# nullmax-vision/SimPB

Measured on AMD Instinct MI355X. Metric: frames/sec (6-cam sample) + MSDeformAttn HBM GB/s, R50 704x256 @1/2/4/8 GPU, higher is better.
Workload: dtype f32

## Files before the change

### include/simpb_hip.h

```cpp
#ifndef SIMPB_HIP_H
#define SIMPB_HIP_H

#ifdef __cplusplus
extern "C" {
#endif

#define SIMPB_OK 0
#define SIMPB_EINVAL 1
#define SIMPB_ELAUNCH 2

#define SIMPB_RECORD3D_WIDTH 15

int simpb_abi_version(void);

const char* simpb_last_error(void);

#define SIMPB_KERNEL_DAF 1
#define SIMPB_KERNEL_MSDA 2
int simpb_timing_enable(int capacity);
int simpb_timing_read(int kernel_id, float* ms_out, int max_n);
void simpb_timing_reset(void);

int simpb_deformable_aggregation_forward(
    float* output, const float* mc_ms_feat, const int* spatial_shape, const int* scale_start_index,
// ... 80 lines not shown
int simpb_preprocess_mid_pitch(int out_width);

#define SIMPB_GEMM_MAX_SEGS 4
#define SIMPB_GEMM_MAX_JOBS 4
#define SIMPB_GEMM_OUT_F32 0
#define SIMPB_GEMM_OUT_SPLIT_HALFS 1
typedef struct simpb_gemm_job {
  const float* x[SIMPB_GEMM_MAX_SEGS];
  int ldx[SIMPB_GEMM_MAX_SEGS];
  int kseg[SIMPB_GEMM_MAX_SEGS];
  int num_seg;
  int M, N, K;
  const float* w;
  const float* bias;
  float* y;
  const int* m_live;
  int ldw, ldy, relu;
  int out_fmt;
  const int* row_flag;
  const float* bias2;
  const void* w_hi;
  const void* w_lo;
} simpb_gemm_job;
typedef struct simpb_gemm_args {
  int num_jobs;
  int reserved;
  simpb_gemm_job job[SIMPB_GEMM_MAX_JOBS];
} simpb_gemm_args;
int simpb_gemm_f32(const simpb_gemm_args* args, void* stream);

int simpb_layernorm_f32(float* out, int ldo, const float* x0, int ld0, int k0, const float* x1, int ld1, int k1,
                        const float* gamma, const float* beta, int num_rows, const int* m_live, void* stream);

#define SIMPB_MAX_LEVELS 8
int simpb_format_tokens(float* col_feats, const void* const* level_ptrs, const void* const* level_bias,
                        const int* level_hw, int num_levels, int num_images, int channels, int src_is_half, void* stream);

int simpb_bias_act_nhwc_f16(void* y, const void* bias, const void* residual, long long num_pixels, int channels,
                            int relu, void* stream);

int simpb_bias_relu_maxpool_nhwc_f16(void* y, const void* x, const void* bias, int num_images, int in_h, int in_w,
                                     int channels, void* stream);

int simpb_conv1x1_nhwc_f16(void* y, const void* x, const void* weight, const void* bias, const void* residual,
                           int num_images, int in_h, int in_w, int in_channels, int out_channels, int stride, int relu,
                           int residual_upsample2x, const void* input_bias, int variant, void* stream);

int simpb_conv3x3_nhwc_f16(void* y, float* tokens, void* tokens_f16, int tokens_per_cam, int level_start, const void* x,
                           const void* weight, const void* bias, int num_images, int in_h, int in_w, int in_channels,
                           int out_channels, int stride, int relu, int variant, void* stream);

int simpb_conv3x3_choose_variant(long long p_out, int in_channels, int out_channels);

int simpb_conv3x3_group_tokens_f16(int num_levels, float* tokens, void* tokens_f16, int tokens_per_cam, const int* level_start,
                                   const void* const* x, const void* const* weight, const void* const* bias, int num_images,
                                   const int* in_h, const int* in_w, int in_channels, int out_channels, int relu, void* stream);

int simpb_attention_f32(float* out, const float* q, const float* k, const float* v, const int* query_cam,
                        const int* group_start, int batch_size, int num_heads, int head_dim, int num_query,
                        int num_key, int ldq, int ldk, int ldv, int ldo, float scale, void* stream);

int simpb_attention_f32_split(float* out, const float* q, const float* k, const float* v, const int* query_cam,
                              const int* group_start, int batch_size, int num_heads, int head_dim, int num_query,
                              int num_key, int ldq, int ldk, int ldv, int ldo, float scale, void* stream);

int simpb_attention_split_halfs(float* out, const void* q, const void* k, const void* v, const int* query_cam,
                                const int* group_start, int batch_size, int num_heads, int head_dim, int num_query,
                                int num_key, int ldq, int ldk, int ldv, int ldo, void* stream);

#define SIMPB_MLP_MAX_OPS 12
#define SIMPB_MLP_MAX_CHAINS 8
#define SIMPB_MLP_POST_NONE 0
#define SIMPB_MLP_POST_REFINE3D 1
#define SIMPB_MLP_POST_REFINE2D 2
#define SIMPB_MLP_POST_SIGMOID 3
#define SIMPB_MLP_LINEAR 0
#define SIMPB_MLP_LAYERNORM 1
#define SIMPB_MLP_IN_ROWS 0
#define SIMPB_MLP_IN_SINE2D 1
#define SIMPB_MLP_IN_ROWS_LN 2
typedef struct simpb_mlp_op {
  int type, in_dim, out_dim, relu;
  const float* w;
  const float* b;
} simpb_mlp_op;
typedef struct simpb_mlp_chain {
  const float* x;
  const float* x2;
  float* out;
  const float* out_scale;
  int ldx, ldx2, ldo, in_dim, in_mode, n_ops;
  int post, ldres, res_cols, div_rows, div_col0, reserved;
  const float* res;
  const float* div;
  simpb_mlp_op ops[SIMPB_MLP_MAX_OPS];
  const float* ln_w;
  const float* ln_b;
  float* ln_out;
  int ld_ln_out, reserved2;
} simpb_mlp_chain;
typedef struct simpb_mlp_args {
  int num_rows, num_chains;
  int weights_transposed;
  int reserved;
  simpb_mlp_chain chain[SIMPB_MLP_MAX_CHAINS];
  const int* m_live;
} simpb_mlp_args;
int simpb_mlp_chain_forward(const simpb_mlp_args* args, void* stream);

// ... 157 lines not shown
```

### simpb_amd/_lib.py

```python
import ctypes
import os

from .build import LIB

_lib = None

_P = ctypes.c_void_p
_I = ctypes.c_int
_F = ctypes.c_float
_LL = ctypes.c_longlong


class WorldTables(ctypes.Structure):
    _fields_ = [("class_range", _F * 32), ("attr_moving", ctypes.c_ubyte * 32), ("attr_still", ctypes.c_ubyte * 32),
                ("threshold", _F), ("has_threshold", _I), ("num_output", _I)]


SIGNATURES = {
    "simpb_abi_version": ([], _I),
    "simpb_last_error": ([], ctypes.c_char_p),
    "simpb_timing_enable": ([_I], _I),
    "simpb_timing_read": ([_I, _P, _I], _I),
    "simpb_timing_reset": ([], None),
    "simpb_deformable_aggregation_forward": ([_P] * 6 + [_I] * 8 + [_P], _I),
    "simpb_dfa_fused_forward": ([_P, _P, _I] + [_P] * 11 + [_I] * 9 + [_P], _I),
    "simpb_dfa_fused_forward_cams": ([_P, _P, _I] + [_P] * 11 + [_I] * 9 + [_P, _P], _I),
    "simpb_deformable_aggregation_backward": ([_P] * 9 + [_I] * 8 + [_P], _I),
    "simpb_ms_deform_attn_grouped_forward": ([_P] * 7 + [_I] * 8 + [_P], _I),
    "simpb_msda_linear_forward": ([_P, _I, _P, _I, _P, _P, _P, _I, _P, _I, _P, _P] + [_I] * 8 + [_P], _I),
    "simpb_ms_deform_attn_grouped_backward": ([_P] * 10 + [_I] * 8 + [_P], _I),
    "simpb_linear_f32": ([_P] * 4 + [_I] * 4 + [_P], _I),
    "simpb_linear_f16x3": ([_P] * 5 + [_I] * 3 + [_P], _I),
    "simpb_gemm_f32": ([_P, _P], _I),
    "simpb_layernorm_f32": ([_P, _I, _P, _I, _I, _P, _I, _I, _P, _P, _I, _P, _P], _I),
    "simpb_bias_act_nhwc_f16": ([_P, _P, _P, ctypes.c_longlong, _I, _I, _P], _I),
    "simpb_bias_relu_maxpool_nhwc_f16": ([_P, _P, _P, _I, _I, _I, _I, _P], _I),
    "simpb_conv1x1_nhwc_f16": ([_P] * 5 + [_I] * 8 + [_P, _I, _P], _I),
    "simpb_conv3x3_nhwc_f16": ([_P, _P, _P, _I, _I, _P, _P, _P] + [_I] * 8 + [_P], _I),
    "simpb_conv3x3_choose_variant": ([_LL, _I, _I], _I),
    "simpb_conv3x3_group_tokens_f16": ([_I, _P, _P, _I, _P, _P, _P, _P, _I, _P, _P, _I, _I, _I, _P], _I),
    "simpb_stem_conv7x7_pool_f16": ([_P] * 4 + [_I] * 4 + [_P], _I),
    "simpb_image_to_nhwc4_f16": ([_P, _P] + [ctypes.c_longlong] * 4 + [_I] * 4 + [_P], _I),
    "simpb_preprocess_u8_nhwc4_f16": ([_P] * 10 + [_I] * 11 + [_P], _I),
    "simpb_preprocess_yuv420sp_nhwc4_f16": ([_P] * 10 + [_I] * 18 + [_P], _I),
    "simpb_preprocess_surface_nhwc4_f16": ([_P] * 11 + [_I] * 12 + [_LL] * 4 + [_I] * 6 + [_P], _I),
    "simpb_preprocess_mid_pitch": ([_I], _I),
    "simpb_linear_f16in_split": ([_P] * 5 + [_I] * 3 + [_P], _I),
    "simpb_format_tokens": ([_P, _P, _P, _P, _I, _I, _I, _I, _P], _I),
    "simpb_attention_f32": ([_P] * 6 + [_I] * 9 + [_F, _P], _I),
    "simpb_attention_f32_split": ([_P] * 6 + [_I] * 9 + [_F, _P], _I),
    "simpb_attention_split_halfs": ([_P] * 6 + [_I] * 9 + [_P], _I),
    "simpb_mlp_chain_forward": ([_P, _P], _I),
    "simpb_bank_get": ([_P] * 6 + [_I] * 2 + [_F] * 2 + [_P], _I),
    "simpb_bank_update": ([_P] * 10 + [_I] * 5 + [_P], _I),
    "simpb_bank_update_rank": ([_P, _P] + [_I] * 4 + [_P], _I),
    "simpb_bank_update_merge": ([_P] * 13 + [_I, _P] + [_I] * 5 + [_P], _I),
    "simpb_bank_update_merge_active": ([_P] * 13 + [_I, _P] + [_I] * 5 + [_P, _P], _I),
    "simpb_bank_cache": ([_P] * 10 + [_I] * 6 + [_F, _I, _F, _P, _I, _P, _P], _I),
    "simpb_bank_cache_streams": ([_P] * 10 + [_I] * 6 + [_F, _I, _F, _P, _I, _P, _P, _P], _I),
    "simpb_bank_cache_streams_active": ([_P] * 10 + [_I] * 6 + [_F, _I, _F, _P, _I, _P, _P, _P, _P], _I),
    "simpb_decode3d_record": ([_P] * 6 + [_I] * 4 + [_P], _I),
    "simpb_decode2d_record": ([_P] * 6 + [_I] * 4 + [_F] * 4 + [_P], _I),
    "simpb_record2d_compact": ([_P, _LL, _P, _LL, _I, _I, _I, _P], _I),
    "simpb_decode2d_record_ragged": ([_P] * 7 + [_I] * 5 + [_F] * 4 + [_P], _I),
    "simpb_world_record": ([_P] * 5 + [WorldTables, _I, _P], _I),
    "simpb_topk_rows": ([_P, _P, _P, _I, _I, _I, _P], _I),
    "simpb_rowdot_sigmoid": ([_P, _P, _I, _P, _P, _I, _I, _P, _P], _I),
    "simpb_anchor_projection": ([_P] * 4 + [_I] * 2 + [_P], _I),
    "simpb_msda_prep": ([_P, _P, _P, _I, _P, _I, _P, _I, _I, _I, _I, _P, _P], _I),
    "simpb_dfa_points": ([_P] * 7 + [_I] * 5 + [_P], _I),
    "simpb_dfa_weights": ([_P] * 3 + [_I] * 6 + [_P], _I),
    "simpb_dfa_points_cams": ([_P] * 7 + [_I] * 5 + [_P, _P], _I),
    "simpb_dfa_weights_cams": ([_P] * 3 + [_I] * 6 + [_P, _P], _I),
    "simpb_alloc_project_cams": ([_P] * 5 + [_I] * 3 + [_F] * 5 + [_P, _P], _I),
    "simpb_alloc_project": ([_P] * 5 + [_I] * 3 + [_F] * 5 + [_P], _I),
    "simpb_alloc_compact": ([_P] * 3 + [_I] * 3 + [_P], _I),
    "simpb_alloc_group_start": ([_P] * 3 + [_I] * 3 + [_P], _I),
    "simpb_alloc_scatter": ([_P] * 12 + [_I] * 4 + [_F] * 2 + [_P], _I),
    "simpb_alloc_static": ([_P] * 15 + [_I] * 4 + [_F] * 5 + [_P], _I),
    "simpb_alloc_ragged": ([_P] * 15 + [_I] * 4 + [_F] * 5 + [_P], _I),
    "simpb_alloc_ragged_active": ([_P] * 15 + [_I] * 4 + [_F] * 5 + [_P, _P], _I),
    "simpb_alloc_static_cams": ([_P] * 15 + [_I] * 4 + [_F] * 5 + [_P, _P], _I),
    "simpb_alloc_ragged_cams": ([_P] * 15 + [_I] * 4 + [_F] * 5 + [_P, _P, _P], _I),
    "simpb_gather_rows": ([_P] * 3 + [_I] * 4 + [_P], _I),
    "simpb_aggregate_2d_to_3d": ([_P] * 8 + [_I] * 5 + [_P], _I),
    "simpb_aggregate_2d_to_3d_alpha": ([_P] * 9 + [_I, _I, _P, _P] + [_I] * 5 + [_P], _I),
}

ERRORS = {1: "SIMPB_EINVAL (bad pointer/size/layout)", 2: "SIMPB_ELAUNCH (kernel launch failed)"}


def lib():
    global _lib
# ... 22 lines not shown
```

### simpb_amd/csrc/conv3x3.hip

```cpp
#include <hip/hip_runtime.h>
#include <hip/hip_fp16.h>
#include <type_traits>
#include "../../include/simpb_hip.h"
#include "mfma_f16.h"

extern "C" int simpb_check_launch(void);

namespace {

using f32x16 = __attribute__((ext_vector_type(16))) float;
using h16x8 = __attribute__((ext_vector_type(8))) _Float16;

constexpr int BN = 64, BK = 64;
constexpr int LDH = BK + 8;
constexpr int LDC = BN + 1;
constexpr int kThreads = 256;
constexpr int kStageBytes = 2 * BN * LDH * 2;
constexpr int kTileBytes = 4 * 32 * LDC * 4;
constexpr int kSmemBytes = kStageBytes > kTileBytes ? kStageBytes : kTileBytes;

struct ConvArgs {
  _Float16* y;
  float* tok;
  _Float16* tok16;
  const _Float16 *x, *w, *bias;
  const _Float16* residual;
  int res_up;
  int P_out, Cin, Cout, relu, stride, Ho, Wo, H, W;
  int tokens_per_cam, level_start;
  int gx, gy, per_xcd;
};

template <int S>
using IC = std::integral_constant<int, S>;

template <bool TOK16>
__device__ __forceinline__ void emit_piece(const ConvArgs& a, int c0, bool full, int p, int c8, const float (&v)[8]) {
  if (p >= a.P_out) return;
  size_t trow = 0;
  if (TOK16 || a.tok) {
    const int hw = a.Ho * a.Wo;
    const int n = p / hw, pix = p - n * hw;
    trow = ((size_t)n * a.tokens_per_cam + a.level_start + pix) * a.Cout;
  }
  size_t rrow = 0;
  if (a.residual) {
    int rp = p;
    if (a.res_up) {
      const int hw = a.Ho * a.Wo;
      const int n = p / hw, rem = p - n * hw;
      const int ho = rem / a.Wo, wo = rem - ho * a.Wo;
      rp = (n * (a.Ho >> 1) + (ho >> 1)) * (a.Wo >> 1) + (wo >> 1);
    }
    rrow = (size_t)rp * a.Cout;
  }
  if (full) {
    const h16x8 bv = *reinterpret_cast<const h16x8*>(a.bias + c0 + c8);
    h16x8 rv = {0, 0, 0, 0, 0, 0, 0, 0};
    if (a.residual) rv = *reinterpret_cast<const h16x8*>(a.residual + rrow + c0 + c8);
    h16x8 o;
#pragma unroll
    for (int e = 0; e < 8; ++e) {
      const float t = v[e] + (float)bv[e] + (float)rv[e];
      o[e] = (_Float16)(a.relu ? fmaxf(t, 0.f) : t);
    }
    if constexpr (TOK16) {
      *reinterpret_cast<h16x8*>(a.tok16 + trow + c0 + c8) = o;
    } else if (a.tok) {
      float* d = a.tok + trow + c0 + c8;
      *reinterpret_cast<float4*>(d) = make_float4((float)o[0], (float)o[1], (float)o[2], (float)o[3]);
      *reinterpret_cast<float4*>(d + 4) = make_float4((float)o[4], (float)o[5], (float)o[6], (float)o[7]);
      if (a.tok16) *reinterpret_cast<h16x8*>(a.tok16 + trow + c0 + c8) = o;
    } else {
      *reinterpret_cast<h16x8*>(a.y + (size_t)p * a.Cout + c0 + c8) = o;
    }
  } else {
#pragma unroll
    for (int e = 0; e < 8; ++e) {
      const int c = c0 + c8 + e;
      if (c < a.Cout) {
        float t = v[e] + (float)a.bias[c];
        if (a.residual) t += (float)a.residual[rrow + c];
        const _Float16 o = (_Float16)(a.relu ? fmaxf(t, 0.f) : t);
// ... 406 lines not shown
}

template <int BMt, int BNt, int WGM, int WGN, int TAPS, bool TOK16>
__global__ __launch_bounds__(64 * WGM * WGN, WGM * WGN == 3 ? 3 : 2) void conv_staged_kernel(const ConvArgs a) {
  const int tile = (blockIdx.x & 7) * a.per_xcd + (blockIdx.x >> 3);
  if ((int)(blockIdx.x >> 3) >= a.per_xcd || tile >= a.gx * a.gy) return;
  conv_staged_tile<BMt, BNt, WGM, WGN, TAPS, TOK16>(a, tile);
}

template <int BMt, int BNt, int WGM, int WGN, int TAPS, bool TOK16, int KS>
__global__ __launch_bounds__(64 * WGM * WGN * KS, 2) void conv_staged_ksplit_kernel(const ConvArgs a) {
  const int tile = (blockIdx.x & 7) * a.per_xcd + (blockIdx.x >> 3);
  if ((int)(blockIdx.x >> 3) >= a.per_xcd || tile >= a.gx * a.gy) return;
  conv_staged_tile<BMt, BNt, WGM, WGN, TAPS, TOK16, KS, true>(a, tile);
}

constexpr int kMaxConvGroup = 4;
struct ConvGroup {
  ConvArgs a[kMaxConvGroup];
  int start[kMaxConvGroup + 1];
  int n, per_xcd;
};
template <int BMt, int BNt, int WGM, int WGN, int TAPS, bool TOK16>
__global__ __launch_bounds__(64 * WGM * WGN, WGM * WGN == 3 ? 3 : 2) void conv_staged_group_kernel(const ConvGroup g) {
  const int gt = (blockIdx.x & 7) * g.per_xcd + (blockIdx.x >> 3);
  if ((int)(blockIdx.x >> 3) >= g.per_xcd || gt >= g.start[g.n]) return;
  int j = 0;
#pragma unroll
  for (int t = 1; t < kMaxConvGroup; ++t)
    if (t < g.n && gt >= g.start[t]) j = t;
  conv_staged_tile<BMt, BNt, WGM, WGN, TAPS, TOK16>(g.a[j], gt - g.start[j]);
}

template <int BMt, int BNt, int WGM, int WGN, int TAPS, bool TOK16>
void launch_staged(ConvArgs& a, hipStream_t stream) {
  a.gx = (a.P_out + BMt - 1) / BMt;
  a.gy = (a.Cout + BNt - 1) / BNt;
  const long long total = (long long)a.gx * a.gy;
  a.per_xcd = (int)((total + 7) / 8);
  hipLaunchKernelGGL((conv_staged_kernel<BMt, BNt, WGM, WGN, TAPS, TOK16>), dim3((unsigned)(a.per_xcd * 8)), dim3(64 * WGM * WGN), 0,
                     stream, a);
}

template <int BMt, int BNt, int WGM, int WGN, int TAPS, bool TOK16, int KS>
void launch_staged_ksplit(ConvArgs& a, hipStream_t stream) {
  a.gx = (a.P_out + BMt - 1) / BMt;
  a.gy = (a.Cout + BNt - 1) / BNt;
  const long long total = (long long)a.gx * a.gy;
  a.per_xcd = (int)((total + 7) / 8);
  hipLaunchKernelGGL((conv_staged_ksplit_kernel<BMt, BNt, WGM, WGN, TAPS, TOK16, KS>), dim3((unsigned)(a.per_xcd * 8)),
                     dim3(64 * WGM * WGN * KS), 0, stream, a);
}

}

extern "C" int simpb_conv3x3_choose_variant(long long p_out, int in_channels, int out_channels) {
  const long long ny = (out_channels + BN - 1) / BN;
  const long long t96 = (p_out + 95) / 96, t128 = (p_out + 127) / 128, t64 = (p_out + 63) / 64;
  if (out_channels >= 128 && t128 * ((out_channels + 127) / 128) >= 2048) return 6;
  if (out_channels >= 128 && t96 * ((out_channels + 127) / 128) >= 160) return 8;
  if (t96 * ny >= 256) return 7;
  if (t128 * ny >= 128) return in_channels >= 256 && out_channels >= 256 ? 9 : 1;
  if (t64 * ny >= 128) return in_channels >= 512 && out_channels >= 512 ? 11 : 4;
  return 3;
}

extern "C" int simpb_conv3x3_nhwc_f16(void* y, float* tokens, void* tokens_f16, int tokens_per_cam, int level_start,
                                      const void* x, const void* weight, const void* bias, int num_images, int in_h, int in_w,
                                      int in_channels, int out_channels, int stride, int relu, int variant, void* stream) {
  const bool to_tokens = tokens || tokens_f16;
  if ((!y && !to_tokens) || (y && to_tokens) || (reinterpret_cast<size_t>(tokens_f16) & 15) || !x || !weight || !bias || num_images <= 0 || in_h <= 0 || in_w <= 0 ||
      in_channels <= 0 || out_channels <= 0 || (stride != 1 && stride != 2) || in_channels % BK != 0 || out_channels % 8 != 0 ||
      variant < 0 || variant > 11)
    return SIMPB_EINVAL;
  if ((reinterpret_cast<size_t>(y) | reinterpret_cast<size_t>(tokens) | reinterpret_cast<size_t>(x) |
       reinterpret_cast<size_t>(weight) | reinterpret_cast<size_t>(bias)) & 15)
    return SIMPB_EINVAL;
  const int ho = (in_h - 1) / stride + 1, wo = (in_w - 1) / stride + 1;
  const long long p_out = (long long)num_images * ho * wo;
  const long long in_elems = (long long)num_images * in_h * in_w * in_channels;
  if (p_out > (1ll << 30) || in_elems > (1ll << 31) - 1) return SIMPB_EINVAL;
  if (to_tokens && (tokens_per_cam < ho * wo || level_start < 0 || level_start + ho * wo > tokens_per_cam)) return SIMPB_EINVAL;
  (void)hipGetLastError();
  ConvArgs a{static_cast<_Float16*>(y), tokens, static_cast<_Float16*>(tokens_f16), static_cast<const _Float16*>(x), static_cast<const _Float16*>(weight),
             static_cast<const _Float16*>(bias), nullptr, 0, (int)p_out, in_channels, out_channels, relu, stride, ho, wo, in_h, in_w,
             tokens_per_cam, level_start, 0, 0, 0};
  if (variant == 0) variant = simpb_conv3x3_choose_variant(p_out, in_channels, out_channels);
  hipStream_t s = static_cast<hipStream_t>(stream);
  auto dispatch = [&](auto tok16_c) {
    constexpr bool T = decltype(tok16_c)::value;
    switch (variant) {
      case 1: launch<1, false, T>(a, s); break;
      case 2: launch<2, false, T>(a, s); break;
      case 3: launch<1, true, T>(a, s); break;
      case 4: launch<2, true, T>(a, s); break;
      case 5: launch_staged<128, 64, 4, 1, 9, T>(a, s); break;
      case 6: launch_staged<128, 128, 2, 2, 9, T>(a, s); break;
      case 7: launch_staged<96, 64, 3, 1, 9, T>(a, s); break;
      case 8: launch_staged<96, 128, 1, 4, 9, T>(a, s); break;
      case 9: launch_staged_ksplit<64, 64, 2, 2, 9, T, 1>(a, s); break;
      case 10: launch_staged_ksplit<64, 64, 2, 2, 9, T, 2>(a, s); break;
      default: launch_staged_ksplit<64, 64, 2, 2, 9, T, 4>(a, s); break;
    }
  };
  if (!tokens && tokens_f16) dispatch(std::true_type{});
  else dispatch(std::false_type{});
  return simpb_check_launch();
}

extern "C" int simpb_conv3x3_group_tokens_f16(int num_levels, float* tokens, void* tokens_f16, int tokens_per_cam,
                                              const int* level_start, const void* const* x, const void* const* weight,
                                              const void* const* bias, int num_images, const int* in_h, const int* in_w,
                                              int in_channels, int out_channels, int relu, void* stream) {
  if (num_levels < 1 || num_levels > kMaxConvGroup || (!tokens && !tokens_f16) || !level_start || !x || !weight || !bias || !in_h || !in_w ||
      num_images <= 0 || in_channels <= 0 || out_channels <= 0 || in_channels % BK != 0 || out_channels % 8 != 0 ||
      ((reinterpret_cast<size_t>(tokens) | reinterpret_cast<size_t>(tokens_f16)) & 15))
    return SIMPB_EINVAL;
  ConvGroup g{};
  long long total = 0;
  for (int j = 0; j < num_levels; ++j) {
    if (!x[j] || !weight[j] || !bias[j] || in_h[j] <= 0 || in_w[j] <= 0 ||
        ((reinterpret_cast<size_t>(x[j]) | reinterpret_cast<size_t>(weight[j]) | reinterpret_cast<size_t>(bias[j])) & 15))
      return SIMPB_EINVAL;
    const long long p_out = (long long)num_images * in_h[j] * in_w[j];
    if (p_out > (1ll << 30) || p_out * in_channels > (1ll << 31) - 1) return SIMPB_EINVAL;
    if (tokens_per_cam < in_h[j] * in_w[j] || level_start[j] < 0 || level_start[j] + in_h[j] * in_w[j] > tokens_per_cam)
      return SIMPB_EINVAL;
    g.a[j] = ConvArgs{nullptr, tokens, static_cast<_Float16*>(tokens_f16), static_cast<const _Float16*>(x[j]),
                      static_cast<const _Float16*>(weight[j]), static_cast<const _Float16*>(bias[j]), nullptr, 0, (int)p_out,
                      in_channels, out_channels, relu, 1, in_h[j], in_w[j], in_h[j], in_w[j], tokens_per_cam, level_start[j],
                      0, 0, 0};
    g.a[j].gx = (int)((p_out + 95) / 96);
    g.a[j].gy = (out_channels + 127) / 128;
    g.start[j] = (int)total;
    total += (long long)g.a[j].gx * g.a[j].gy;
  }
  if (total > (1 << 24)) return SIMPB_EINVAL;
  for (int j = num_levels; j <= kMaxConvGroup; ++j) g.start[j] = (int)total;
  g.n = num_levels;
  g.per_xcd = (int)((total + 7) / 8);
  (void)hipGetLastError();
  if (!tokens)
    hipLaunchKernelGGL((conv_staged_group_kernel<96, 128, 1, 4, 9, true>), dim3((unsigned)(g.per_xcd * 8)), dim3(256), 0,
                       static_cast<hipStream_t>(stream), g);
  else
    hipLaunchKernelGGL((conv_staged_group_kernel<96, 128, 1, 4, 9, false>), dim3((unsigned)(g.per_xcd * 8)), dim3(256), 0,
                       static_cast<hipStream_t>(stream), g);
  return simpb_check_launch();
}

extern "C" int simpb_conv_pointwise_staged(void* y, const void* x, const void* weight, const void* bias, const void* residual,
                                           int p_out, int in_h, int in_w, int ho, int wo, int in_channels, int out_channels,
                                           int stride, int relu, int residual_upsample2x, int tiling, void* stream) {
  ConvArgs a{static_cast<_Float16*>(y), nullptr, nullptr, static_cast<const _Float16*>(x), static_cast<const _Float16*>(weight),
             static_cast<const _Float16*>(bias), static_cast<const _Float16*>(residual), residual_upsample2x ? 1 : 0,
             p_out, in_channels, out_channels, relu, stride, ho, wo, in_h, in_w, 0, 0, 0, 0, 0};
  hipStream_t s = static_cast<hipStream_t>(stream);
  if (tiling == 0) launch_staged<128, 64, 4, 1, 1, false>(a, s);
  else if (tiling == 1) launch_staged<128, 128, 2, 2, 1, false>(a, s);
  else launch_staged<64, 64, 2, 2, 1, false>(a, s);
  return simpb_check_launch();
}
```

### simpb_amd/plugin/ops.py

```python
import ctypes

import torch
from torch.autograd.function import Function

from .. import _lib


def _ptr(t):
    return ctypes.c_void_p(t.data_ptr())


def _stream():
    return ctypes.c_void_p(torch.cuda.current_stream().cuda_stream)


def _require_gpu(*tensors):
    for t in tensors:
        if not t.is_cuda:
            raise RuntimeError("simpb_amd operators run on the GPU only (got a CPU tensor); "
                               "there is no CPU fallback")


_layout_ok = {}

# ... 399 lines not shown
        raise ValueError("residual must match the output (channels_last f16)")
    if input_bias is not None and (input_bias.dtype != torch.float16 or input_bias.numel() != cin or not input_bias.is_contiguous()):
        raise ValueError("input_bias must be a contiguous f16 [Cin] tensor")
    w2 = weight.reshape(cout, cin)
    if not w2.is_contiguous():
        w2 = w2.contiguous()
    status = _lib.lib().simpb_conv1x1_nhwc_f16(_ptr(y), _ptr(x), _ptr(w2), _ptr(bias), _ptr(residual) if residual is not None else None,
                                               n, h, w, cin, cout, stride, 1 if relu else 0,
                                               1 if residual_upsample2x else 0,
                                               _ptr(input_bias) if input_bias is not None else None, variant, _stream())
    _lib.check(status, "simpb_conv1x1_nhwc_f16")
    return y


def conv3x3_nhwc(x, weight, bias, relu=True, stride=1, tokens=None, variant=0):
    _require_gpu(x, weight, bias)
    n, cin, h, w = x.shape
    cout = weight.shape[0]
    if (x.dtype != torch.float16 or not x.is_contiguous(memory_format=torch.channels_last) or weight.dtype != torch.float16
            or bias.dtype != torch.float16 or tuple(weight.shape) != (cout, cin, 3, 3) or cin % 64 or cout % 8
            or stride not in (1, 2) or bias.numel() != cout or not bias.is_contiguous()):
        raise ValueError("conv3x3_nhwc takes channels_last f16 input, f16 [Cout, Cin, 3, 3] weight, Cin % 64 == 0, Cout % 8 == 0")
    if not weight.is_contiguous(memory_format=torch.channels_last):
        weight = weight.contiguous(memory_format=torch.channels_last)
    ho, wo = (h - 1) // stride + 1, (w - 1) // stride + 1
    col16 = None
    if tokens is None:
        y = torch.empty((n, cout, ho, wo), device=x.device, dtype=torch.float16, memory_format=torch.channels_last)
        col, per_cam, start = None, 0, 0
    else:
        col, per_cam, start = tokens[:3]
        col16 = tokens[3] if len(tokens) > 3 else None
        y = None
        if col is None and col16 is None:
            raise ValueError("tokens: an f32 or an f16 token buffer")
        if col16 is not None and (col16.dtype != torch.float16 or not col16.is_contiguous()
                                  or (col is not None and col16.shape != col.shape)):
            raise ValueError("tokens: the f16 buffer must match col_feats")
        rows = col if col is not None else col16
        if ((col is not None and col.dtype != torch.float32) or not rows.is_contiguous() or rows.shape[-1] != cout
                or rows.numel() != n * per_cam * cout or start < 0 or start + ho * wo > per_cam):
            raise ValueError("tokens: (contiguous f32 [bs, cams * tokens_per_cam, Cout] with bs * cams == N, tokens_per_cam, level_start)")
    status = _lib.lib().simpb_conv3x3_nhwc_f16(_ptr(y) if y is not None else None, _ptr(col) if col is not None else None,
                                               _ptr(col16) if col16 is not None else None, per_cam, start, _ptr(x), _ptr(weight), _ptr(bias), n, h, w, cin, cout, stride,
                                               1 if relu else 0, variant, _stream())
    _lib.check(status, "simpb_conv3x3_nhwc_f16")
    return y


def conv3x3_variant_for(p_out, in_channels, out_channels):
    return int(_lib.lib().simpb_conv3x3_choose_variant(int(p_out), int(in_channels), int(out_channels)))


def conv3x3_group_tokens(xs, weights, biases, col, per_cam, starts, col16=None, relu=False):
    import ctypes
    if col is None and col16 is None:
        raise ValueError("conv3x3_group_tokens: an f32 or an f16 token buffer")
    rows = col if col is not None else col16
    _require_gpu(*xs, *weights, *biases, rows)
    n, cin = xs[0].shape[:2]
    cout = weights[0].shape[0]
    k = len(xs)
    if not (1 <= k <= 4 and len(weights) == k and len(biases) == k and len(starts) == k):
        raise ValueError("conv3x3_group_tokens: 1..4 levels, one weight / bias / start each")
    ws = []
    for x, w, b in zip(xs, weights, biases):
        if (x.dtype != torch.float16 or not x.is_contiguous(memory_format=torch.channels_last) or x.shape[0] != n or x.shape[1] != cin
                or w.dtype != torch.float16 or tuple(w.shape) != (cout, cin, 3, 3) or b.dtype != torch.float16 or b.numel() != cout
                or not b.is_contiguous() or cin % 64 or cout % 8):
            raise ValueError("conv3x3_group_tokens takes channels_last f16 inputs of one channel count, f16 [Cout, Cin, 3, 3] weights")
        ws.append(w if w.is_contiguous(memory_format=torch.channels_last) else w.contiguous(memory_format=torch.channels_last))
    if ((col is not None and col.dtype != torch.float32) or not rows.is_contiguous() or rows.shape[-1] != cout
            or rows.numel() != n * per_cam * cout
            or (col16 is not None and (col16.dtype != torch.float16 or not col16.is_contiguous() or col16.shape != rows.shape))):
        raise ValueError("conv3x3_group_tokens: col = contiguous f32 [bs, cams * tokens_per_cam, Cout] with bs * cams == N")
    arr_p, arr_i = ctypes.c_void_p * k, ctypes.c_int * k
    status = _lib.lib().simpb_conv3x3_group_tokens_f16(
        k, _ptr(col) if col is not None else None, _ptr(col16) if col16 is not None else None, int(per_cam), arr_i(*[int(v) for v in starts]),
        arr_p(*[x.data_ptr() for x in xs]), arr_p(*[w.data_ptr() for w in ws]), arr_p(*[b.data_ptr() for b in biases]), n,
        arr_i(*[x.shape[2] for x in xs]), arr_i(*[x.shape[3] for x in xs]), cin, cout, 1 if relu else 0, _stream())
    _lib.check(status, "simpb_conv3x3_group_tokens_f16")


def _stem_weight_packed(weight):
    tag = (weight.data_ptr(), weight._version, str(weight.device))
    hit = getattr(weight, "_simpb_stem_pack", None)
    if hit is None or hit[0] != tag:
        with torch.no_grad():
            w = weight.detach().float()
            full = torch.zeros(64, 4, 7, 8, device=w.device)
            full[:, :3, :, :7] = w
            pack = full.reshape(64, 4, 7, 4, 2).permute(2, 3, 4, 0, 1).contiguous().half()
        hit = (tag, pack)
        weight._simpb_stem_pack = hit
    return hit[1]


def stem_conv_pool(img, weight, bias):
    _require_gpu(img, weight, bias)
    n, c, h, w = img.shape
    if img.dtype != torch.float32 or c != 3 or tuple(weight.shape) != (64, 3, 7, 7) or bias.numel() != 64 or h < 1 or w < 1:
        raise ValueError("stem_conv_pool: f32 [N, 3, H, W] image, [64, 3, 7, 7] weight, 64 biases")
    lib = _lib.lib()
    x4 = torch.empty(n, h, w, 4, device=img.device, dtype=torch.float16)
    _lib.check(lib.simpb_image_to_nhwc4_f16(_ptr(x4), _ptr(img), img.stride(0), img.stride(1), img.stride(2), img.stride(3), n, c, h, w,
                                            _stream()), "simpb_image_to_nhwc4_f16")
    return stem_conv_pool_nhwc4(x4, weight, bias)


def stem_conv_pool_nhwc4(x4, weight, bias):
    _require_gpu(x4, weight, bias)
    if (x4.dtype != torch.float16 or x4.dim() != 4 or x4.shape[3] != 4 or not x4.is_contiguous() or tuple(weight.shape) != (64, 3, 7, 7)
            or bias.numel() != 64 or x4.shape[1] < 1 or x4.shape[2] < 1):
        raise ValueError("stem_conv_pool_nhwc4: contiguous f16 [N, H, W, 4] image, [64, 3, 7, 7] weight, 64 biases")
    n, h, w, _ = x4.shape
    lib = _lib.lib()
    ho, wo = (h - 1) // 2 + 1, (w - 1) // 2 + 1
    hp, wp = (ho - 1) // 2 + 1, (wo - 1) // 2 + 1
    out = torch.empty((n, 64, hp, wp), device=x4.device, dtype=torch.float16, memory_format=torch.channels_last)
    b16 = bias if bias.dtype == torch.float16 and bias.is_contiguous() else bias.half().contiguous()
    _lib.check(lib.simpb_stem_conv7x7_pool_f16(_ptr(out), _ptr(x4), _ptr(_stem_weight_packed(weight)), _ptr(b16), n, h, w, 64,
                                               _stream()), "simpb_stem_conv7x7_pool_f16")
    return out


def preprocess_frames(frames, plan, out=None):
    return plan.run(frames, out=out)


def topk_rows(scores, k):
    _require_gpu(scores)
    if scores.dim() != 2 or scores.shape[1] > 2048:
        raise ValueError("topk_rows takes [bs, n <= 2048] scores")
    scores = scores.contiguous().float()
# ... 47 lines not shown
```

Baseline: 429.0.

## Add LDS-resident halo-tile conv3x3 kernel with per-level group dispatch

Adds a new conv3x3 implicit-GEMM kernel that loads a spatial tile with its halo and the full input-channel depth into LDS once, then reuses it across all nine taps while streaming weight chunks through a 2-3 deep LDS ring. The group-tokens path now picks between this resident form and the existing staged kernel per level, using a heuristic based on tile count, and launches up to two kernels. The aim is to stop re-reading overlapping input pixels from global memory for every tap. The cost is heavy LDS use, which can lower occupancy, plus an extra launch when levels are split between the two forms.

```diff
diff --git a/include/simpb_hip.h b/include/simpb_hip.h
--- a/include/simpb_hip.h
+++ b/include/simpb_hip.h
@@ -156,9 +156,19 @@
 
 int simpb_conv3x3_choose_variant(long long p_out, int in_channels, int out_channels);
 
+int simpb_conv3x3_choose_resident(long long p_out, int in_h, int in_w, int in_channels, int out_channels, int stride);
+
+int simpb_conv3x3_group_choose_resident(int num_levels, int num_images, const int* in_h, const int* in_w, int in_channels,
+                                        int out_channels);
+
 int simpb_conv3x3_group_tokens_f16(int num_levels, float* tokens, void* tokens_f16, int tokens_per_cam, const int* level_start,
                                    const void* const* x, const void* const* weight, const void* const* bias, int num_images,
                                    const int* in_h, const int* in_w, int in_channels, int out_channels, int relu, void* stream);
+
+int simpb_conv3x3_group_tokens_forms_f16(int num_levels, float* tokens, void* tokens_f16, int tokens_per_cam,
+                                         const int* level_start, const void* const* x, const void* const* weight,
+                                         const void* const* bias, int num_images, const int* in_h, const int* in_w,
+                                         int in_channels, int out_channels, int relu, const int* variant, void* stream);
 
 int simpb_attention_f32(float* out, const float* q, const float* k, const float* v, const int* query_cam,
                         const int* group_start, int batch_size, int num_heads, int head_dim, int num_query,
diff --git a/simpb_amd/_lib.py b/simpb_amd/_lib.py
--- a/simpb_amd/_lib.py
+++ b/simpb_amd/_lib.py
@@ -39,6 +39,9 @@
     "simpb_conv3x3_nhwc_f16": ([_P, _P, _P, _I, _I, _P, _P, _P] + [_I] * 8 + [_P], _I),
     "simpb_conv3x3_choose_variant": ([_LL, _I, _I], _I),
     "simpb_conv3x3_group_tokens_f16": ([_I, _P, _P, _I, _P, _P, _P, _P, _I, _P, _P, _I, _I, _I, _P], _I),
+    "simpb_conv3x3_choose_resident": ([_LL, _I, _I, _I, _I, _I], _I),
+    "simpb_conv3x3_group_choose_resident": ([_I, _I, _P, _P, _I, _I], _I),
+    "simpb_conv3x3_group_tokens_forms_f16": ([_I, _P, _P, _I, _P, _P, _P, _P, _I, _P, _P, _I, _I, _I, _P, _P], _I),
     "simpb_stem_conv7x7_pool_f16": ([_P] * 4 + [_I] * 4 + [_P], _I),
     "simpb_image_to_nhwc4_f16": ([_P, _P] + [ctypes.c_longlong] * 4 + [_I] * 4 + [_P], _I),
     "simpb_preprocess_u8_nhwc4_f16": ([_P] * 10 + [_I] * 11 + [_P], _I),
diff --git a/simpb_amd/csrc/conv3x3.hip b/simpb_amd/csrc/conv3x3.hip
--- a/simpb_amd/csrc/conv3x3.hip
+++ b/simpb_amd/csrc/conv3x3.hip
@@ -29,6 +29,7 @@
   int P_out, Cin, Cout, relu, stride, Ho, Wo, H, W;
   int tokens_per_cam, level_start;
   int gx, gy, per_xcd;
+  int tiles_w, tiles_h;
 };
 
 template <int S>
@@ -541,6 +542,281 @@
                      dim3(64 * WGM * WGN * KS), 0, stream, a);
 }
 
+constexpr int RTW = 16, RHW = RTW + 2;
+constexpr int resident_row_bytes(int cin) { return (RHW * (2 * cin + 16) + 255) & ~255; }
+
+template <int CIN, int TH, int BNt, int WGM, int WGN, int RING>
+constexpr size_t resident_lds() {
+  const size_t run = (size_t)(TH + 2) * resident_row_bytes(CIN) + RING * BNt * LDH * 2;
+  const size_t tile = (size_t)WGM * WGN * 32 * (BNt / WGN + 1) * 4;
+  return run > tile ? run : tile;
+}
+
+template <int CIN, int TH, int BNt, int WGM, int WGN, int RING, bool TOK16>
+__device__ __forceinline__ void conv_resident_tile(const ConvArgs& a, const int tile, unsigned char* smem) {
+  constexpr int NT = 64 * WGM * WGN;
+  constexpr int AF = TH * RTW / WGM / 32, NF = BNt / WGN / 32;
+  static_assert(AF * WGM * 32 == TH * RTW && NF * WGN * 32 == BNt && NF <= 2, "tile = waves x 32-row / 32-column fragments");
+  static_assert(CIN == 64 || CIN == 128 || CIN == 256, "the whole Cin is resident");
+  static_assert(RING == 2 || RING == 3, "weight chunks in LDS");
+  constexpr int D = RING - 1;
+  constexpr int PT = CIN / BK, NCH = 9 * PT;
+  constexpr int HEAD = PT <= 2 ? 3 : 6;
+  constexpr int NB = (BNt * 8 + NT - 1) / NT;
+  constexpr int LDW = 32 * NF + 1;
+  constexpr int HP = (TH + 2) * RHW;
+  constexpr int NH = (HP * 8 + NT - 1) / NT;
+  constexpr int PIX = 2 * CIN + 16, ROW = resident_row_bytes(CIN);
+  constexpr int WBUF = BNt * LDH;
+  _Float16* s_b = reinterpret_cast<_Float16*>(smem + (TH + 2) * ROW);
+  float* s_c = reinterpret_cast<float*>(smem);
+  const int W = a.W, H = a.H;
+
+  const int tx = tile / a.gy, ty = tile - tx * a.gy;
+  const int per_img = a.tiles_w * a.tiles_h;
+  const int img = tx / per_img, t2 = tx - img * per_img;
+  const int trow = t2 / a.tiles_w;
+  const int y0 = trow * TH, x0 = (t2 - trow * a.tiles_w) * RTW;
+  const int tid = threadIdx.x;
+  const int lane = tid & 63, wave = tid >> 6;
+  const int r32 = lane & 31, kb = lane >> 5;
+  const int wm = wave / WGN, wn = wave - wm * WGN;
+  const int c0 = ty * BNt;
+  constexpr size_t K = (size_t)9 * CIN;
+  const _Float16* __restrict__ wgt = a.w;
+  const h16x8 zero = {0, 0, 0, 0, 0, 0, 0, 0};
+
+  const int sc = (tid & 7) * 8;
+  size_t brow[NB];
+#pragma unroll
+  for (int i = 0; i < NB; ++i) brow[i] = (size_t)min(c0 + ((tid + NT * i) >> 3), a.Cout - 1) * K + sc;
+  h16x8 rb[3][NB];
+  auto fetch = [&](auto set_c, int chunk) __attribute__((always_inline)) {
+    constexpr int s = decltype(set_c)::value;
+    const size_t koff = (size_t)min(chunk, NCH - 1) * BK;
+#pragma unroll
+    for (int i = 0; i < NB; ++i) rb[s][i] = *reinterpret_cast<const h16x8*>(wgt + brow[i] + koff);
+  };
+  auto stash = [&](auto set_c, int buf) __attribute__((always_inline)) {
+    constexpr int s = decltype(set_c)::value;
+#pragma unroll
+    for (int i = 0; i < NB; ++i) {
+      const int idx = tid + NT * i;
+      if ((BNt * 8) % NT == 0 || idx < BNt * 8) *reinterpret_cast<h16x8*>(&s_b[buf * WBUF + (idx >> 3) * LDH + sc]) = rb[s][i];
+    }
+  };
+
+  fetch(IC<0>{}, 0);
+  fetch(IC<1>{}, 1);
+  fetch(IC<2>{}, 2);
+  h16x8 hv[PT][NH];
+  {
+    const _Float16* __restrict__ src = a.x + (size_t)img * H * W * CIN;
+#pragma unroll
+    for (int i = 0; i < NH; ++i) {
+      const int idx = tid + NT * i;
+      const int hp = idx >> 3;
+      const int hy = hp / RHW, hx = hp - hy * RHW;
+      const int iy = y0 - 1 + hy, ix = x0 - 1 + hx;
+      const bool in = ((HP * 8) % NT == 0 || idx < HP * 8) && iy >= 0 && iy < H && ix >= 0 && ix < W;
+      const _Float16* from = src + ((size_t)iy * W + ix) * CIN + sc;
+#pragma unroll
+      for (int s = 0; s < PT; ++s) {
+        hv[s][i] = zero;
+        if (in) hv[s][i] = *reinterpret_cast<const h16x8*>(from + s * BK);
+      }
+    }
+  }
+  auto halo_to_lds = [&](auto slice_c) __attribute__((always_inline)) {
+    constexpr int s = decltype(slice_c)::value;
+#pragma unroll
+    for (int i = 0; i < NH; ++i) {
+      const int idx = tid + NT * i;
+      const int hp = idx >> 3;
+      const int hy = hp / RHW, hx = hp - hy * RHW;
+      if ((HP * 8) % NT == 0 || idx < HP * 8) *reinterpret_cast<h16x8*>(smem + hy * ROW + hx * PIX + s * (2 * BK) + 2 * sc) = hv[s][i];
+    }
+  };
+  __builtin_amdgcn_sched_barrier(0);
+  stash(IC<0>{}, 0);
+  fetch(IC<0>{}, 3);
+  if constexpr (D == 2) {
+    stash(IC<1>{}, 1);
+    fetch(IC<1>{}, 4);
+  }
+  halo_to_lds(IC<0>{});
+  __syncthreads();
+
+  f32x16 acc[AF][NF];
+#pragma unroll
+  for (int f = 0; f < AF; ++f)
+#pragma unroll
+    for (int n = 0; n < NF; ++n)
+#pragma unroll
+      for (int r = 0; r < 16; ++r) acc[f][n][r] = 0.f;
+
+  const unsigned char* a_lane = smem + (wm * AF * 2 + (r32 >> 4)) * ROW + (r32 & 15) * PIX + 16 * kb;
+  const _Float16* b_lane = s_b + (wn * NF * 32 + r32) * LDH + 8 * kb;
+  h16x8 av[AF], bv[NF];
+  auto pixels = [&](int c, int ks) __attribute__((always_inline)) {
+    const int tap = c / PT, k0 = (c - tap * PT) * BK;
+    const int dy = tap / 3, dx = tap - dy * 3;
+    const unsigned char* sa = a_lane + dy * ROW + dx * PIX + 2 * k0 + 32 * ks;
+#pragma unroll
+    for (int f = 0; f < AF; ++f) av[f] = *reinterpret_cast<const h16x8*>(sa + f * 2 * ROW);
+  };
+  auto weights = [&](int c, int ks) __attribute__((always_inline)) {
+    const _Float16* sb = b_lane + (c % RING) * WBUF + 16 * ks;
+#pragma unroll
+    for (int n = 0; n < NF; ++n) bv[n] = *reinterpret_cast<const h16x8*>(sb + n * 32 * LDH);
+  };
+  auto step = [&](auto set_c, int c, bool ahead, bool read_ahead) __attribute__((always_inline)) {
+    stash(set_c, (c + D) % RING);
+    fetch(set_c, c + D + 3);
+    if constexpr (PT > 1) {
+      if (c == 0) halo_to_lds(IC<1>{});
+    }
+    if constexpr (PT > 2) {
+      if (c == 1) halo_to_lds(IC<2>{});
+      if (c == 2) halo_to_lds(IC<3>{});
+    }
+    __builtin_amdgcn_sched_barrier(0);
+    if (!ahead) pixels(c, 0);
+    if (!ahead || D == 1) weights(c, 0);
+#pragma unroll
+    for (int ks = 0; ks < BK / 16; ++ks) {
+      h16x8 ca[AF], cb[NF];
+#pragma unroll
+      for (int f = 0; f < AF; ++f) ca[f] = av[f];
+#pragma unroll
+      for (int n = 0; n < NF; ++n) cb[n] = bv[n];
+      if (ks + 1 < BK / 16) {
+        pixels(c, ks + 1);
+        weights(c, ks + 1);
+      } else if (read_ahead) {
+        pixels(min(c + 1, NCH - 1), 0);
+        if constexpr (D == 2) weights(min(c + 1, NCH - 1), 0);
+      }
+#pragma unroll
+      for (int f = 0; f < AF; ++f)
+#pragma unroll
+        for (int n = 0; n < NF; ++n) acc[f][n] = simpb::mfma_32x32x16_f16(ca[f], cb[n], acc[f][n]);
+    }
+    __syncthreads();
+  };
+  using S0 = IC<D % 3>;
+  using S1 = IC<(D + 1) % 3>;
+  using S2 = IC<(D + 2) % 3>;
+  step(S0{}, 0, false, 1 >= PT);
+  step(S1{}, 1, 1 >= PT, 2 >= PT);
+  step(S2{}, 2, 2 >= PT, 3 >= PT);
+  if constexpr (HEAD == 6) {
+    step(S0{}, 3, 3 >= PT, true);
+    step(S1{}, 4, true, true);
+    step(S2{}, 5, true, true);
+  }
+  for (int c = HEAD; c < NCH; c += 3) {
+    step(S0{}, c, true, true);
+    step(S1{}, c + 1, true, true);
+    step(S2{}, c + 2, true, true);
+  }
+
+  float* mine = s_c + wave * 32 * LDW;
+  const int cw = c0 + wn * NF * 32;
+  const bool full = cw + 32 * NF <= a.Cout;
+#pragma unroll
+  for (int f = 0; f < AF; ++f) {
+    if (f) __syncthreads();
+#pragma unroll
+    for (int n = 0; n < NF; ++n)
+#pragma unroll
+      for (int r = 0; r < 16; ++r) mine[((r & 3) + 8 * (r >> 2) + 4 * kb) * LDW + n * 32 + r32] = acc[f][n][r];
+    __syncthreads();
+    constexpr int PR = 4 * NF;
+#pragma unroll
+    for (int pass = 0; pass < 32 * PR / 64; ++pass) {
+      const int idx = lane + 64 * pass;
+      const int r = idx / PR, c8 = (idx % PR) * 8;
+      float v[8];
+#pragma unroll
+      for (int e = 0; e < 8; ++e) v[e] = mine[r * LDW + c8 + e];
+      const int oy = y0 + (wm * AF + f) * 2 + (r >> 4), ox = x0 + (r & 15);
+      const int p = oy < H && ox < W ? (img * H + oy) * W + ox : a.P_out;
+      emit_piece<TOK16>(a, cw, full, p, c8, v);
+    }
+  }
+}
+
+template <int CIN, int TH, int BNt, int WGM, int WGN, int RING, bool TOK16>
+__global__ __launch_bounds__(64 * WGM * WGN) void conv_resident_kernel(const ConvArgs a) {
+  extern __shared__ __attribute__((aligned(16))) unsigned char resident_smem[];
+  const int tile = (blockIdx.x & 7) * a.per_xcd + (blockIdx.x >> 3);
+  if ((int)(blockIdx.x >> 3) >= a.per_xcd || tile >= a.gx * a.gy) return;
+  conv_resident_tile<CIN, TH, BNt, WGM, WGN, RING, TOK16>(a, tile, resident_smem);
+}
+
+template <int CIN, int TH, int BNt, int WGM, int WGN, int RING, bool TOK16>
+__global__ __launch_bounds__(64 * WGM * WGN) void conv_resident_group_kernel(const ConvGroup g) {
+  extern __shared__ __attribute__((aligned(16))) unsigned char resident_smem[];
+  const int gt = (blockIdx.x & 7) * g.per_xcd + (blockIdx.x >> 3);
+  if ((int)(blockIdx.x >> 3) >= g.per_xcd || gt >= g.start[g.n]) return;
+  int j = 0;
+#pragma unroll
+  for (int t = 1; t < kMaxConvGroup; ++t)
+    if (t < g.n && gt >= g.start[t]) j = t;
+  conv_resident_tile<CIN, TH, BNt, WGM, WGN, RING, TOK16>(g.a[j], gt - g.start[j], resident_smem);
+}
+
+inline bool resident_shape(int cin, int stride) { return stride == 1 && (cin == 64 || cin == 128 || cin == 256); }
+
+template <int TH, int BNt>
+void resident_grid(ConvArgs& a) {
+  a.tiles_w = (a.Wo + RTW - 1) / RTW;
+  a.tiles_h = (a.Ho + TH - 1) / TH;
+  a.gx = a.P_out / (a.Ho * a.Wo) * a.tiles_w * a.tiles_h;
+  a.gy = (a.Cout + BNt - 1) / BNt;
+}
+
+template <typename KernelT>
+bool allow_resident_lds(KernelT kernel, size_t bytes) {
+  return hipFuncSetAttribute(reinterpret_cast<const void*>(kernel), hipFuncAttributeMaxDynamicSharedMemorySize, (int)bytes) == hipSuccess;
+}
+
+template <int CIN, int TH, int BNt, int WGM, int WGN, int RING, bool TOK16>
+void launch_resident_cin(ConvArgs& a, hipStream_t stream) {
+  constexpr size_t lds = resident_lds<CIN, TH, BNt, WGM, WGN, RING>();
+  auto kernel = conv_resident_kernel<CIN, TH, BNt, WGM, WGN, RING, TOK16>;
+  static const bool allowed = allow_resident_lds(kernel, lds);
+  (void)allowed;
+  resident_grid<TH, BNt>(a);
+  const long long total = (long long)a.gx * a.gy;
+  a.per_xcd = (int)((total + 7) / 8);
+  hipLaunchKernelGGL(kernel, dim3((unsigned)(a.per_xcd * 8)), dim3(64 * WGM * WGN), lds, stream, a);
+}
+
+template <int TH, int BNt, int WGM, int WGN, int RING, bool TOK16>
+void launch_resident(ConvArgs& a, hipStream_t stream) {
+  if (a.Cin == 64) launch_resident_cin<64, TH, BNt, WGM, WGN, RING, TOK16>(a, stream);
+  else if (a.Cin == 128) launch_resident_cin<128, TH, BNt, WGM, WGN, RING, TOK16>(a, stream);
+  else launch_resident_cin<256, TH, BNt, WGM, WGN, RING, TOK16>(a, stream);
+}
+
+template <int CIN, int TH, int BNt, int WGM, int WGN, int RING, bool TOK16>
+void launch_resident_group_cin(const ConvGroup& g, hipStream_t stream) {
+  constexpr size_t lds = resident_lds<CIN, TH, BNt, WGM, WGN, RING>();
+  auto kernel = conv_resident_group_kernel<CIN, TH, BNt, WGM, WGN, RING, TOK16>;
+  static const bool allowed = allow_resident_lds(kernel, lds);
+  (void)allowed;
+  hipLaunchKernelGGL(kernel, dim3((unsigned)(g.per_xcd * 8)), dim3(64 * WGM * WGN), lds, stream, g);
+}
+
+template <int TH, int BNt, int WGM, int WGN, int RING, bool TOK16>
+void launch_resident_group(const ConvGroup& g, hipStream_t stream) {
+  if (g.a[0].Cin == 64) launch_resident_group_cin<64, TH, BNt, WGM, WGN, RING, TOK16>(g, stream);
+  else if (g.a[0].Cin == 128) launch_resident_group_cin<128, TH, BNt, WGM, WGN, RING, TOK16>(g, stream);
+  else launch_resident_group_cin<256, TH, BNt, WGM, WGN, RING, TOK16>(g, stream);
+}
+
 }
 
 extern "C" int simpb_conv3x3_choose_variant(long long p_out, int in_channels, int out_channels) {
@@ -554,14 +830,40 @@
   return 3;
 }
 
+extern "C" int simpb_conv3x3_choose_resident(long long p_out, int in_h, int in_w, int in_channels, int out_channels, int stride) {
+  if (p_out <= 0 || in_h <= 0 || in_w <= 0 || p_out % ((long long)in_h * in_w) != 0 || !resident_shape(in_channels, stride) ||
+      out_channels != in_channels)
+    return 0;
+  const int staged = simpb_conv3x3_choose_variant(p_out, in_channels, out_channels);
+  if (staged != 7 && staged != 8) return 0;
+  const long long images = p_out / ((long long)in_h * in_w), across = (in_w + RTW - 1) / RTW;
+  const long long t13 = images * ((in_h + 7) / 8) * across * ((out_channels + 127) / 128);
+  const long long t12 = images * ((in_h + 3) / 4) * across * ((out_channels + 63) / 64);
+  if (in_channels == 256 && t13 >= 1024) return 13;
+  if (t12 >= 512) return 12;
+  return 0;
+}
+
+extern "C" int simpb_conv3x3_group_choose_resident(int num_levels, int num_images, const int* in_h, const int* in_w, int in_channels,
+                                                   int out_channels) {
+  if (num_levels < 1 || num_levels > kMaxConvGroup || num_images <= 0 || !in_h || !in_w || in_channels != 256 || out_channels != 256) return 0;
+  long long tiles = 0;
+  for (int j = 0; j < num_levels; ++j) {
+    if (in_h[j] <= 0 || in_w[j] <= 0) return 0;
+    tiles += (long long)num_images * ((in_h[j] + 7) / 8) * ((in_w[j] + RTW - 1) / RTW) * 2;
+  }
+  return tiles >= 1024 ? 13 : 0;
+}
+
 extern "C" int simpb_conv3x3_nhwc_f16(void* y, float* tokens, void* tokens_f16, int tokens_per_cam, int level_start,
                                       const void* x, const void* weight, const void* bias, int num_images, int in_h, int in_w,
                                       int in_channels, int out_channels, int stride, int relu, int variant, void* stream) {
   const bool to_tokens = tokens || tokens_f16;
   if ((!y && !to_tokens) || (y && to_tokens) || (reinterpret_cast<size_t>(tokens_f16) & 15) || !x || !weight || !bias || num_images <= 0 || in_h <= 0 || in_w <= 0 ||
       in_channels <= 0 || out_channels <= 0 || (stride != 1 && stride != 2) || in_channels % BK != 0 || out_channels % 8 != 0 ||
-      variant < 0 || variant > 11)
+      variant < 0 || variant > 13)
     return SIMPB_EINVAL;
+  if (variant >= 12 && !resident_shape(in_channels, stride)) return SIMPB_EINVAL;
   if ((reinterpret_cast<size_t>(y) | reinterpret_cast<size_t>(tokens) | reinterpret_cast<size_t>(x) |
        reinterpret_cast<size_t>(weight) | reinterpret_cast<size_t>(bias)) & 15)
     return SIMPB_EINVAL;
@@ -574,7 +876,13 @@
   ConvArgs a{static_cast<_Float16*>(y), tokens, static_cast<_Float16*>(tokens_f16), static_cast<const _Float16*>(x), static_cast<const _Float16*>(weight),
              static_cast<const _Float16*>(bias), nullptr, 0, (int)p_out, in_channels, out_channels, relu, stride, ho, wo, in_h, in_w,
              tokens_per_cam, level_start, 0, 0, 0};
-  if (variant == 0) variant = simpb_conv3x3_choose_variant(p_out, in_channels, out_channels);
+  if (variant == 0) {
+    variant = simpb_conv3x3_choose_variant(p_out, in_channels, out_channels);
+    if (variant == 7 || variant == 8) {
+      const int resident = simpb_conv3x3_choose_resident(p_out, in_h, in_w, in_channels, out_channels, stride);
+      if (resident) variant = resident;
+    }
+  }
   hipStream_t s = static_cast<hipStream_t>(stream);
   auto dispatch = [&](auto tok16_c) {
     constexpr bool T = decltype(tok16_c)::value;
@@ -589,7 +897,9 @@
       case 8: launch_staged<96, 128, 1, 4, 9, T>(a, s); break;
       case 9: launch_staged_ksplit<64, 64, 2, 2, 9, T, 1>(a, s); break;
       case 10: launch_staged_ksplit<64, 64, 2, 2, 9, T, 2>(a, s); break;
-      default: launch_staged_ksplit<64, 64, 2, 2, 9, T, 4>(a, s); break;
+      case 11: launch_staged_ksplit<64, 64, 2, 2, 9, T, 4>(a, s); break;
+      case 12: launch_resident<4, 64, 2, 2, 2, T>(a, s); break;
+      default: launch_resident<8, 128, 4, 2, 3, T>(a, s); break;
     }
   };
   if (!tokens && tokens_f16) dispatch(std::true_type{});
@@ -597,16 +907,17 @@
   return simpb_check_launch();
 }
 
-extern "C" int simpb_conv3x3_group_tokens_f16(int num_levels, float* tokens, void* tokens_f16, int tokens_per_cam,
-                                              const int* level_start, const void* const* x, const void* const* weight,
-                                              const void* const* bias, int num_images, const int* in_h, const int* in_w,
-                                              int in_channels, int out_channels, int relu, void* stream) {
+extern "C" int simpb_conv3x3_group_tokens_forms_f16(int num_levels, float* tokens, void* tokens_f16, int tokens_per_cam,
+                                                    const int* level_start, const void* const* x, const void* const* weight,
+                                                    const void* const* bias, int num_images, const int* in_h, const int* in_w,
+                                                    int in_channels, int out_channels, int relu, const int* variant, void* stream) {
   if (num_levels < 1 || num_levels > kMaxConvGroup || (!tokens && !tokens_f16) || !level_start || !x || !weight || !bias || !in_h || !in_w ||
       num_images <= 0 || in_channels <= 0 || out_channels <= 0 || in_channels % BK != 0 || out_channels % 8 != 0 ||
       ((reinterpret_cast<size_t>(tokens) | reinterpret_cast<size_t>(tokens_f16)) & 15))
     return SIMPB_EINVAL;
-  ConvGroup g{};
-  long long total = 0;
+  ConvGroup form[2] = {};
+  long long total[2] = {0, 0};
+  const int rule = variant ? 0 : simpb_conv3x3_group_choose_resident(num_levels, num_images, in_h, in_w, in_channels, out_channels);
   for (int j = 0; j < num_levels; ++j) {
     if (!x[j] || !weight[j] || !bias[j] || in_h[j] <= 0 || in_w[j] <= 0 ||
         ((reinterpret_cast<size_t>(x[j]) | reinterpret_cast<size_t>(weight[j]) | reinterpret_cast<size_t>(bias[j])) & 15))
@@ -615,27 +926,49 @@
     if (p_out > (1ll << 30) || p_out * in_channels > (1ll << 31) - 1) return SIMPB_EINVAL;
     if (tokens_per_cam < in_h[j] * in_w[j] || level_start[j] < 0 || level_start[j] + in_h[j] * in_w[j] > tokens_per_cam)
       return SIMPB_EINVAL;
-    g.a[j] = ConvArgs{nullptr, tokens, static_cast<_Float16*>(tokens_f16), static_cast<const _Float16*>(x[j]),
-                      static_cast<const _Float16*>(weight[j]), static_cast<const _Float16*>(bias[j]), nullptr, 0, (int)p_out,
-                      in_channels, out_channels, relu, 1, in_h[j], in_w[j], in_h[j], in_w[j], tokens_per_cam, level_start[j],
-                      0, 0, 0};
-    g.a[j].gx = (int)((p_out + 95) / 96);
-    g.a[j].gy = (out_channels + 127) / 128;
-    g.start[j] = (int)total;
-    total += (long long)g.a[j].gx * g.a[j].gy;
-  }
-  if (total > (1 << 24)) return SIMPB_EINVAL;
-  for (int j = num_levels; j <= kMaxConvGroup; ++j) g.start[j] = (int)total;
-  g.n = num_levels;
-  g.per_xcd = (int)((total + 7) / 8);
+    const int v = variant ? variant[j] : rule ? rule : 8;
+    if (v != 8 && v != 13) return SIMPB_EINVAL;
+    if (v == 13 && !resident_shape(in_channels, 1)) return SIMPB_EINVAL;
+    const int f = v == 13;
+    ConvGroup& g = form[f];
+    ConvArgs& a = g.a[g.n];
+    a = ConvArgs{nullptr, tokens, static_cast<_Float16*>(tokens_f16), static_cast<const _Float16*>(x[j]),
+                 static_cast<const _Float16*>(weight[j]), static_cast<const _Float16*>(bias[j]), nullptr, 0, (int)p_out,
+                 in_channels, out_channels, relu, 1, in_h[j], in_w[j], in_h[j], in_w[j], tokens_per_cam, level_start[j],
+                 0, 0, 0, 0, 0};
+    if (f == 1) {
+      resident_grid<8, 128>(a);
+    } else {
+      a.gx = (int)((p_out + 95) / 96);
+      a.gy = (out_channels + 127) / 128;
+    }
+    g.start[g.n++] = (int)total[f];
+    total[f] += (long long)a.gx * a.gy;
+  }
+  for (int f = 0; f < 2; ++f) {
+    if (total[f] > (1 << 24)) return SIMPB_EINVAL;
+    for (int j = form[f].n; j <= kMaxConvGroup; ++j) form[f].start[j] = (int)total[f];
+    form[f].per_xcd = (int)((total[f] + 7) / 8);
+  }
   (void)hipGetLastError();
-  if (!tokens)
-    hipLaunchKernelGGL((conv_staged_group_kernel<96, 128, 1, 4, 9, true>), dim3((unsigned)(g.per_xcd * 8)), dim3(256), 0,
-                       static_cast<hipStream_t>(stream), g);
-  else
-    hipLaunchKernelGGL((conv_staged_group_kernel<96, 128, 1, 4, 9, false>), dim3((unsigned)(g.per_xcd * 8)), dim3(256), 0,
-                       static_cast<hipStream_t>(stream), g);
+  hipStream_t s = static_cast<hipStream_t>(stream);
+  auto launches = [&](auto tok16_c) {
+    constexpr bool T = decltype(tok16_c)::value;
+    if (form[1].n) launch_resident_group<8, 128, 4, 2, 3, T>(form[1], s);
+    if (form[0].n)
+      hipLaunchKernelGGL((conv_staged_group_kernel<96, 128, 1, 4, 9, T>), dim3((unsigned)(form[0].per_xcd * 8)), dim3(256), 0, s, form[0]);
+  };
+  if (!tokens) launches(std::true_type{});
+  else launches(std::false_type{});
   return simpb_check_launch();
+}
+
+extern "C" int simpb_conv3x3_group_tokens_f16(int num_levels, float* tokens, void* tokens_f16, int tokens_per_cam,
+                                              const int* level_start, const void* const* x, const void* const* weight,
+                                              const void* const* bias, int num_images, const int* in_h, const int* in_w,
+                                              int in_channels, int out_channels, int relu, void* stream) {
+  return simpb_conv3x3_group_tokens_forms_f16(num_levels, tokens, tokens_f16, tokens_per_cam, level_start, x, weight, bias, num_images,
+                                              in_h, in_w, in_channels, out_channels, relu, nullptr, stream);
 }
 
 extern "C" int simpb_conv_pointwise_staged(void* y, const void* x, const void* weight, const void* bias, const void* residual,
diff --git a/simpb_amd/plugin/ops.py b/simpb_amd/plugin/ops.py
--- a/simpb_amd/plugin/ops.py
+++ b/simpb_amd/plugin/ops.py
@@ -475,7 +475,18 @@
     return int(_lib.lib().simpb_conv3x3_choose_variant(int(p_out), int(in_channels), int(out_channels)))
 
 
-def conv3x3_group_tokens(xs, weights, biases, col, per_cam, starts, col16=None, relu=False):
+def conv3x3_resident_for(p_out, in_h, in_w, in_channels, out_channels, stride=1):
+    return int(_lib.lib().simpb_conv3x3_choose_resident(int(p_out), int(in_h), int(in_w), int(in_channels), int(out_channels), int(stride)))
+
+
+def conv3x3_group_resident_for(num_images, hws, in_channels, out_channels):
+    import ctypes
+    arr = ctypes.c_int * len(hws)
+    return int(_lib.lib().simpb_conv3x3_group_choose_resident(len(hws), int(num_images), arr(*[int(h) for h, _ in hws]), arr(*[int(w) for _, w in hws]),
+                                                              int(in_channels), int(out_channels)))
+
+
+def conv3x3_group_tokens(xs, weights, biases, col, per_cam, starts, col16=None, relu=False, variants=None):
     import ctypes
     if col is None and col16 is None:
         raise ValueError("conv3x3_group_tokens: an f32 or an f16 token buffer")
@@ -498,11 +509,14 @@
             or (col16 is not None and (col16.dtype != torch.float16 or not col16.is_contiguous() or col16.shape != rows.shape))):
         raise ValueError("conv3x3_group_tokens: col = contiguous f32 [bs, cams * tokens_per_cam, Cout] with bs * cams == N")
     arr_p, arr_i = ctypes.c_void_p * k, ctypes.c_int * k
-    status = _lib.lib().simpb_conv3x3_group_tokens_f16(
+    if variants is not None and len(variants) != k:
+        raise ValueError("conv3x3_group_tokens: one variant per level")
+    status = _lib.lib().simpb_conv3x3_group_tokens_forms_f16(
         k, _ptr(col) if col is not None else None, _ptr(col16) if col16 is not None else None, int(per_cam), arr_i(*[int(v) for v in starts]),
         arr_p(*[x.data_ptr() for x in xs]), arr_p(*[w.data_ptr() for w in ws]), arr_p(*[b.data_ptr() for b in biases]), n,
-        arr_i(*[x.shape[2] for x in xs]), arr_i(*[x.shape[3] for x in xs]), cin, cout, 1 if relu else 0, _stream())
-    _lib.check(status, "simpb_conv3x3_group_tokens_f16")
+        arr_i(*[x.shape[2] for x in xs]), arr_i(*[x.shape[3] for x in xs]), cin, cout, 1 if relu else 0,
+        arr_i(*[int(v) for v in variants]) if variants is not None else None, _stream())
+    _lib.check(status, "simpb_conv3x3_group_tokens_forms_f16")
 
 
 def _stem_weight_packed(weight):
```

After: 443.3, median of 6. 3.3% higher.
